# author-hidden-name/GAN-segmentation

Measured on AMD Instinct MI355X. Metric: synthetic (image,mask) pairs/sec, FFHQ-1024 StyleGAN+decoder, higher is better.
Workload: dtype f32; 1 GPU; stylegan-ffhq 1024^2 synthesis + 2-class decoder, batch=8 per GPU, fp32 (BASELINE.json configs[1]); synthetic weights/latents/noise; (img u8, mask u8) resident on rank 0; global_batch=8, parallelism=dp1, gather=none, backend=none, graph=eager (GSA_GRAPH=0)

## Files before the change

### gan-segmentation_amd/csrc/gsa_dev.h

```cpp
#pragma once
#include "gsa_kernels.h"

#ifndef GSA_NO_XCD_REMAP
#define GSA_NO_XCD_REMAP 0
#endif

namespace gsa {

#ifdef GSA_STAMP
#define GSA_DBG_HOOKS 1
#endif
#ifdef GSA_STAMP
#define STAMP(i) do { __builtin_amdgcn_sched_barrier(0); asm volatile("s_memtime %0\n\ts_waitcnt lgkmcnt(0)" : "=s"(stamp_t[i]) :: "memory"); __builtin_amdgcn_sched_barrier(0); } while (0)
#define STAMP_DECL unsigned long long stamp_t[8] = {0, 0, 0, 0, 0, 0, 0, 0}
#define STAMP_FLUSH(nph) do { if (p.stamps && (threadIdx.x & 63) == 0) { for (int i_ = 0; i_ < (nph); ++i_) atomicAdd(&p.stamps[i_], stamp_t[i_ + 1] - stamp_t[i_]); atomicAdd(&p.stamps[15], 1ull); } } while (0)
#define TICK(var) do { __builtin_amdgcn_sched_barrier(0); asm volatile("s_memtime %0\n\ts_waitcnt lgkmcnt(0)" : "=s"(var) :: "memory"); __builtin_amdgcn_sched_barrier(0); } while (0)
#define TSUM(acc, a, b) acc += (b) - (a)
#define TFLUSH(idx, acc) do { if (p.stamps && (threadIdx.x & 63) == 0) atomicAdd(&p.stamps[idx], acc); } while (0)
#else
#define TICK(var) do {} while (0)
#define TSUM(acc, a, b) do {} while (0)
#define TFLUSH(idx, acc) do {} while (0)
#define STAMP(i) do {} while (0)
#define STAMP_DECL do {} while (0)
// ... 99 lines not shown
__device__ __forceinline__ void loads_landed(f32x4 (&r)[2][2]) { asm("" : GSA_LANDED_2(r[0]), GSA_LANDED_2(r[1])); }
__device__ __forceinline__ void loads_landed(f32x4 (&r)[2], f32x4& pin) { asm("" : GSA_LANDED_2(r), "+v"(pin)); }
__device__ __forceinline__ void loads_landed(f32x4 (&r)[3], f32x4& pin) { asm("" : GSA_LANDED_3(r), "+v"(pin)); }
__device__ __forceinline__ void loads_landed(f32x4 (&r)[6], f32x4& pin) { asm("" : GSA_LANDED_6(r), "+v"(pin)); }
__device__ __forceinline__ void loads_landed(f32x4 (&r)[1][2], f32x4& pin) { asm("" : GSA_LANDED_2(r[0]), "+v"(pin)); }
__device__ __forceinline__ void loads_landed(f32x4 (&r)[2][2], f32x4& pin) { asm("" : GSA_LANDED_2(r[0]), GSA_LANDED_2(r[1]), "+v"(pin)); }
__device__ __forceinline__ void vmem_drained(f32x4& pin) {
    asm volatile("" : "+v"(pin));
    __builtin_amdgcn_s_waitcnt(0x0F70);
}
#undef GSA_LANDED_6
#undef GSA_LANDED_3
#undef GSA_LANDED_2
#undef GSA_LANDED_1

__device__ __forceinline__ f32x2 pk_mul2(f32x2 a, f32x2 b) { f32x2 r; asm("v_pk_mul_f32 %0, %1, %2" : "=v"(r) : "v"(a), "v"(b)); return r; }
__device__ __forceinline__ f32x2 pk_mul2_lo(f32x2 a, f32x2 b) { f32x2 r; asm("v_pk_mul_f32 %0, %1, %2 op_sel_hi:[1,0]" : "=v"(r) : "v"(a), "v"(b)); return r; }
__device__ __forceinline__ f32x2 pk_mul2_hi(f32x2 a, f32x2 b) { f32x2 r; asm("v_pk_mul_f32 %0, %1, %2 op_sel:[0,1]" : "=v"(r) : "v"(a), "v"(b)); return r; }
__device__ __forceinline__ f32x4 fma4(const f32x4& a, const f32x4& m, const f32x4& b) {
    const f32x2 lo = fma2v(a.xy, m.xy, b.xy), hi = fma2v(a.zw, m.zw, b.zw);
    return f32x4{lo.x, lo.y, hi.x, hi.y};
}
__device__ __forceinline__ f32x4 lrelu4(const f32x4& v, f32x2 k02) {
    const f32x2 lo = pk_mul2(v.xy, k02), hi = pk_mul2(v.zw, k02);
    return f32x4{max1(v.x, lo.x), max1(v.y, lo.y), max1(v.z, hi.x), max1(v.w, hi.y)};
}

typedef unsigned u32x2 __attribute__((ext_vector_type(2)));

__device__ __forceinline__ float bf16_lo(unsigned u) { return __uint_as_float(u << 16); }
// ... 31 lines not shown
```

### gan-segmentation_amd/csrc/gsa_sub_lean.hip

```cpp
#include "gsa_kernels.h"
#include "gsa_dev.h"

#include <cstdio>
#include <cstdlib>
#include <type_traits>

namespace gsa {
namespace lean {

constexpr int SLW = 10, SRS = SLW * 16 + 4;
constexpr int SIMG = 10 * SRS;
constexpr int SSEG = 16 * 256;
constexpr int STS = 256;

struct STile { int n, y0, x0; };

__device__ __forceinline__ void settle8(f32x4& a, f32x4& b, f32x4& c, f32x4& d, f32x4& e, f32x4& f, f32x4& g, f32x4& h) {
    asm("s_nop 1" : "+v"(a), "+v"(b), "+v"(c), "+v"(d), "+v"(e), "+v"(f), "+v"(g), "+v"(h));
}
__device__ __forceinline__ void settle5(f32x4& a, f32x4& b, f32x4& c, f32x4& d, f32x4& e) { asm("s_nop 1" : "+v"(a), "+v"(b), "+v"(c), "+v"(d), "+v"(e)); }
__device__ __forceinline__ void mfma_settle9(f32x4 (&a)[9]) {
    asm("s_nop 7\n\ts_nop 3" : "+v"(a[0]), "+v"(a[1]), "+v"(a[2]), "+v"(a[3]), "+v"(a[4]), "+v"(a[5]), "+v"(a[6]), "+v"(a[7]), "+v"(a[8]));
}

// ... 80 lines not shown
            const bool aff = AFF && cb < nblk0;
            if (aff) {
                const float* tab = sC + (t.n & 1) * (nblk0 * 32) + cb * 32 + part * 4;
                kA = *reinterpret_cast<const f32x4*>(tab);
                kB = *reinterpret_cast<const f32x4*>(tab + 16);
            }
#pragma unroll
            for (int k = 0; k < 2; ++k) {
                f32x4 v = aff ? fma4(ra[kb][k], kA, kB) : ra[kb][k];
                if (e && ((eflags >> (4 * k)) & (unsigned)e)) v = z;
                if (k == 0 || l_off[1] >= 0) *reinterpret_cast<f32x4*>(img + l_off[k]) = v;
            }
        }
    };

    auto dma_block = [&](int cbk, int slot) {
#pragma unroll
        for (int j = 0; j < 2 * NT; ++j) {
            const int pc = wave8 + 8 * j, q = pc >> 4, r = pc & 15;
            __builtin_amdgcn_global_load_lds((const __attribute__((address_space(1))) void*)(p.wpk + ((size_t)(g * NT + q) * nblk + cbk) * SSEG + r * 256 + lane * 4),
                                             (__attribute__((address_space(3))) void*)(sW + (slot * NT + q) * SSEG + r * 256), 16, 0, 0);
        }
        if (SC && wave8 < NT)
            __builtin_amdgcn_global_load_lds((const __attribute__((address_space(1))) void*)(p.wsc + ((size_t)(g * NT + wave8) * nblk + cbk) * STS + lane * 4),
                                             (__attribute__((address_space(3))) void*)(sS + (slot * NT + wave8) * STS), 16, 0, 0);
    };
    if (WST) {
        dma_block(0, 0);
    } else {
        for (int i = threadIdx.x; i < nblk * NT * (SSEG / 4); i += 512) {
            const int cbk = i / (NT * (SSEG / 4)), r = i % (NT * (SSEG / 4)), q = r / (SSEG / 4), o = r % (SSEG / 4);
            reinterpret_cast<f32x4*>(sW)[i] = reinterpret_cast<const f32x4*>(p.wpk + ((size_t)(g * NT + q) * nblk + cbk) * SSEG)[o];
        }
        if (SC)
            for (int i = threadIdx.x; i < nblk * NT * (STS / 4); i += 512) {
                const int cbk = i / (NT * (STS / 4)), r = i % (NT * (STS / 4)), q = r / (STS / 4), o = r % (STS / 4);
                reinterpret_cast<f32x4*>(sS)[i] = reinterpret_cast<const f32x4*>(p.wsc + ((size_t)(g * NT + q) * nblk + cbk) * STS)[o];
            }
    }
// ... 85 lines not shown
#pragma unroll
                for (int b = 0; b < 2; ++b) {
                    f32x4 v = y[a][b];
                    if (EPI == EPI_DEC) v = lrelu4(fma4(v, e2[nt], e3[nt]), k02);
                    *reinterpret_cast<f32x4*>(ob + ((long)(2 * a) * W + 2 * b) * COUT * 4 + nt * 64 + lane_out) = v;
                }
            if constexpr (SC) {
                char* sb = reinterpret_cast<char*>(p.out_sc) +
                           (((long)(t.n * Hs + (t.y0 >> 1) + (wave >> 1) * 4) * Ws + (t.x0 >> 1) + (wave & 1) * 4) * COUT + g * 16 * NT + nt * 16) * 4;
                f32x4 sv[1] = {accs[nt]};
                asm("s_nop 7\n\ts_nop 3" : "+v"(sv[0]));
                *reinterpret_cast<f32x4*>(sb + lane_sc) = add4(sv[0], scb[nt]);
            }
        }
    };

    STile tc, tr;
    {
        const int w0 = min(w_begin, p.total_tiles - 1);
        const int tx = w0 % p.tiles_x, r = w0 / p.tiles_x;
        tc.x0 = tx * 16; tc.y0 = (r % p.tiles_y) * 16; tc.n = r / p.tiles_y;
    }
    int ec = edge_code(tc), er, cic = 0, cir = 0, n_tab = tc.n;
    auto next_item = [&](STile& t, int& e, int& ci) {
        if (++ci == nitem) { ci = 0; advance(t); e = edge_code(t); }
    };
    if (AFF) fill_coefficients(tc.n);
    if (total_items > 0) load_item(tc, ec, 0);
    if (WST) asm volatile("s_waitcnt vmcnt(0)" ::: "memory");
    if (CNT && t8 < 8) sCnt[t8] = t8 < 4 ? 1u : 0u;
// ... 98 lines not shown
    const int nblk0 = q.C0 / 16, nblk = (q.C0 + q.C1) / 16, wblk = wst ? 2 : nblk;
    return sizeof(float) * ((size_t)wblk * nt * SSEG + (sc ? (size_t)wblk * nt * STS : 0) + 2 * (cnt ? 3 : 2) * kb * SIMG +
                            (aff ? (cnt ? 8 : 2) * 2 * nblk0 * 32 : 0)) + (cnt ? 64 : 0);
}

bool sub_counters(const ConvParams& q, int nt, bool sc, int kb, bool wst) {
#if GSA_EXPERIMENTS
    static const bool cnt_on = env_int("GSA_SUB_CNT", 0) != 0;
    return cnt_on && !wst && sub_lds(q, nt, sc, q.aff0 != nullptr, kb, false, true) <= 160 * 1024;
#else
    (void)q; (void)nt; (void)sc; (void)kb; (void)wst;
    return false;
#endif
}

template <int NT, int EPI, bool SC, bool AFF, int KB, bool WST, bool CNT = false>
hipError_t launch_k(const ConvParams& q, dim3 grid, hipStream_t s) {
    const size_t lds = sub_lds(q, NT, SC, AFF, KB, WST, CNT);
    if (lds > 160 * 1024) return hipErrorInvalidValue;
    return launch<subpixel_lean<NT, EPI, SC, AFF, KB, WST, CNT>>(q.device, grid, dim3(512), lds, s, q);
}

template <int NT, int EPI, bool SC, bool AFF>
hipError_t launch_shape(const ConvParams& q, int kb, bool wst, dim3 grid, hipStream_t s) {
    if (wst) return launch_k<NT, EPI, SC, AFF, 1, true>(q, grid, s);
#if GSA_EXPERIMENTS
    if (sub_counters(q, NT, SC, kb, false))
        return kb == 2 ? launch_k<NT, EPI, SC, AFF, 2, false, true>(q, grid, s) : launch_k<NT, EPI, SC, AFF, 1, false, true>(q, grid, s);
#endif
    return kb == 2 ? launch_k<NT, EPI, SC, AFF, 2, false>(q, grid, s) : launch_k<NT, EPI, SC, AFF, 1, false>(q, grid, s);
}

}

// ... 3 lines not shown
    if (p.aff0 != nullptr && p.C1 != 0) return false;
    return lean::sub_lds(p, nt, sc, p.aff0 != nullptr, kb, wst, false) <= 160 * 1024;
}

hipError_t launch_subpixel_lean(const ConvParams& q, int nt, int epi, bool sc, int kb, bool wst, dim3 grid, hipStream_t s) {
    using namespace lean;
    const bool aff = q.aff0 != nullptr;
#define GSA_SL(NT, EPI, SC) \
    if (nt == NT && epi == EPI && sc == SC) return aff ? launch_shape<NT, EPI, SC, true>(q, kb, wst, grid, s) : launch_shape<NT, EPI, SC, false>(q, kb, wst, grid, s);
    GSA_SL(1, EPI_RAW, false) GSA_SL(2, EPI_RAW, false) GSA_SL(1, EPI_DEC, false) GSA_SL(2, EPI_DEC, false) GSA_SL(1, EPI_DEC, true) GSA_SL(2, EPI_DEC, true)
#undef GSA_SL
    return hipErrorInvalidValue;
}

}
```

### gan-segmentation_amd/csrc/gsa_wino_lean.hip

```cpp
#include "gsa_kernels.h"
#include "gsa_dev.h"

#include <cstdio>
#include <cstdlib>
#include <type_traits>

namespace gsa {
namespace lean {

constexpr int LH = 18, LW = 18, RS = LW * 16 + 4;
constexpr int IMG = LH * RS;
constexpr int SEG = 16 * 256;
constexpr int NPIX = LH * LW;

struct Tile { int n, y0, x0; };

template <int EPI, bool AFF, bool RES, int NB, int GW, bool DB = true, int PF = 1, bool RGB = false>
__global__ __launch_bounds__(256 * GW, GW == 1 ? (DB ? 2 : 3) : 1) void conv3x3_wino_lean(ConvParams p) {
    static_assert(!RGB || (NB == 1 && GW == 1 && DB && AFF && EPI == EPI_DEC), "fused toRGB: the 16 -> 16 decoder kernel with an AdaIN source");
    static_assert(DB || (NB == 1 && GW == 1), "single-buffered form: one block, one group");
    static_assert(PF == 1 || (PF == 2 && DB), "two prefetch sets: the double-buffered form");
    constexpr int NTHR = 256 * GW, CIN = 16 * NB, COUT = 16 * GW;
    constexpr int NCH = (NPIX * 4 + NTHR - 1) / NTHR;
    constexpr bool kLastPartial = (NPIX * 4) % NTHR != 0;
// ... 404 lines not shown
    antiphase_start(p.group_minor, sC);
#endif

    unsigned s_off[NCH], eflags = 0;
    int l_off[NCH];
#pragma unroll
    for (int k = 0; k < NCH; ++k) {
        const int pix = (tid + NTHR * k) >> 2;
        const bool real = pix < NPIX;
        const int ly = real ? pix / LW : 1, lx = real ? pix % LW : 1;
        s_off[k] = (unsigned)(((ly * W + lx) * CIN + part * 4) * 4);
        l_off[k] = real ? ly * RS + lx * 16 + part * 4 : -1;
        eflags |= (unsigned)((ly == 0 ? 1 : 0) | (ly == LH - 1 ? 2 : 0) | (lx == 0 ? 4 : 0) | (lx == LW - 1 ? 8 : 0)) << (4 * k);
    }
    const unsigned safe_off = (unsigned)((((W + 1) * CIN) + part * 4) * 4);
    auto edge_code = [&](const Tile& t) { return (t.y0 == 0 ? 1 : 0) | (t.y0 + 16 == H ? 2 : 0) | (t.x0 == 0 ? 4 : 0) | (t.x0 + 16 == W ? 8 : 0); };
    auto advance = [&](Tile& t) { t.x0 += 16; if (t.x0 == W) { t.x0 = 0; t.y0 += 16; if (t.y0 == H) { t.y0 = 0; t.n += 1; } } };

    f32x4 ra[NCH];
    int dbg_items = 0; (void)dbg_items;
    const float* const wgrp = p.wpk + (size_t)g * NT * nblk * SEG + lane * 4;
    auto dma_weights = [&](int cb, int buf) {
#ifdef GSA_DBG_HOOKS
        if (p.dbg & 16) cb = 0;
        if ((p.dbg & 1024) && dbg_items > 2) return;
#endif
#pragma unroll
        for (int ct = 0; ct < NT; ++ct) {
            const float* wb = wgrp + ((size_t)ct * nblk + cb) * SEG;
#pragma unroll
            for (int j = 0; j < 4; ++j) {
                const int piece = wave + 4 * j;
                __builtin_amdgcn_global_load_lds((const __attribute__((address_space(1))) void*)(wb + piece * 256),
                                                 (__attribute__((address_space(3))) void*)(sB + (PAIR ? buf * 2 + quad : buf * NT + ct) * SEG + piece * 256), 16, 0, 0);
            }
        }
    };
    auto load_item = [&](const Tile& t, int e, int cb) {
        const char* hb = reinterpret_cast<const char*>(p.src0) + ((((long)(t.n * H + t.y0) * W + t.x0) - (W + 1)) * CIN + cb * 16) * 4;
#ifdef GSA_DBG_HOOKS
        if (p.dbg & 32) hb = reinterpret_cast<const char*>(p.src0) + ((long)(W + 1) * CIN) * 4;
        if ((p.dbg & 512) && dbg_items > 2) return;
#endif
        if (e) {
#pragma unroll
            for (int k = 0; k < NCH; ++k) {
                const unsigned bad = (eflags >> (4 * k)) & (unsigned)e;
                const unsigned off = s_off[k] + (bad ? safe_off - s_off[k] : 0u);
                ra[k] = *reinterpret_cast<const f32x4*>(hb + off);
            }
        } else {
#pragma unroll
            for (int k = 0; k < NCH; ++k) ra[k] = *reinterpret_cast<const f32x4*>(hb + s_off[k]);
        }
    };
    int n_coef = -1;
    auto coefficients = [&](int n) {
        __syncthreads();
        for (int e = tid; e < CIN; e += NTHR) {
            const f32x4 a = *reinterpret_cast<const f32x4*>(p.aff0 + (size_t)n * CIN + e);
            sC[(e >> 4) * 32 + (e & 15)] = a[1];
            sC[(e >> 4) * 32 + 16 + (e & 15)] = a[2];
        }
        __syncthreads();
    };
    auto write_item = [&](const Tile& t, int e, int cb, int buf) {
        float* img = sA + buf * IMG;
        if (AFF && t.n != n_coef) { coefficients(t.n); n_coef = t.n; }
#ifdef GSA_DBG_HOOKS
        if (++dbg_items > 2 && (p.dbg & 128)) return;
#endif
        f32x4 kA = {0.f, 0.f, 0.f, 0.f}, kB = kA;
        if (AFF) {
            kA = *reinterpret_cast<const f32x4*>(sC + cb * 32 + part * 4);
            kB = *reinterpret_cast<const f32x4*>(sC + cb * 32 + 16 + part * 4);
        }
        const f32x4 z = {0.f, 0.f, 0.f, 0.f};
        if (e) {
#pragma unroll
            for (int k = 0; k < NCH; ++k) {
                const f32x4 v = AFF ? fma4(ra[k], kA, kB) : ra[k];
                const bool bad = ((eflags >> (4 * k)) & (unsigned)e) != 0;
                if (k < NCH - 1 || l_off[NCH - 1] >= 0) *reinterpret_cast<f32x4*>(img + l_off[k]) = bad ? z : v;
            }
        } else {
#pragma unroll
            for (int k = 0; k < NCH; ++k)
                if (k < NCH - 1 || l_off[NCH - 1] >= 0) *reinterpret_cast<f32x4*>(img + l_off[k]) = AFF ? fma4(ra[k], kA, kB) : ra[k];
        }
    };

    const int wty = ((i16 >> 3) & 1) * 2 + ((i16 >> 1) & 1), wtx = ((i16 >> 2) & 1) * 2 + (i16 & 1);
    const int qy = wave >> 1, qx = wave & 1;
    const int pbase = (qy * 8 + 2 * wty) * RS + (qx * 8 + 2 * wtx) * 16 + kq * 4;
    const int bbase = (kq * 16 + i16) * 4;
    const int co4 = g * NT * 16 + kq * 4;
    const unsigned out_off = (unsigned)((((qy * 8 + 2 * wty) * W + qx * 8 + 2 * wtx) * COUT + co4) * 4);
    if (tid < 16 * NP) {
        float* e = sE + (tid >> 4) * 64 + (tid & 15);
        const int co = (int)blockIdx.y * NP * 16 + tid;
        e[0] = EPI == EPI_SYNTH ? p.nscale[co] : 0.f;
        e[16] = EPI == EPI_SYNTH ? p.nbias[co] : 0.f;
        e[32] = EPI == EPI_DEC ? p.bn_s[co] : 0.f;
        e[48] = EPI == EPI_DEC ? p.bn_beta[co] : 0.f;
    }
    const unsigned nz_off = (unsigned)((((qy * 8 + 2 * wty) * W + qx * 8 + 2 * wtx)) * 4);
    f32x2 nz[2] = {{0.f, 0.f}, {0.f, 0.f}};
    const int s2 = stat_s2(H * W);
    const bool odd = (lane & 1) != 0;
    unsigned long long dI1[NT][4], dI2[NT][4];
#pragma unroll
    for (int ct = 0; ct < NT; ++ct)
#pragma unroll
        for (int c = 0; c < 4; ++c) dI1[ct][c] = dI2[ct][c] = 0ull;
    auto flush_stats = [&](int n) {
#pragma unroll
        for (int ct = 0; ct < NT; ++ct)
#pragma unroll
            for (int c = 0; c < 4; ++c) {
                unsigned long long I1 = dI1[ct][c], I2 = dI2[ct][c];
#pragma unroll
                for (int m = 1; m < 16; m <<= 1) { I1 += shfl_xor_u64(I1, m); I2 += shfl_xor_u64(I2, m); }
                if (i16 == 0) {
                    StatPart* a = p.partials + ((size_t)n * p.prow + (blockIdx.x & (kDirectRows - 1))) * COUT + co4 + ct * 16 + c;
                    atomicAdd(&a->s1, I1);
                    atomicAdd(&a->s2, I2);
                }
                dI1[ct][c] = dI2[ct][c] = 0ull;
            }
    };
    const f32x2 k02 = {0.2f, 0.2f};
    auto epilogue_loads = [&](const Tile& t) {
        if (EPI == EPI_SYNTH) {
            const char* nb = reinterpret_cast<const char*>(p.noise) + ((long)(t.n * H + t.y0) * W + t.x0) * 4;
            nz[0] = *reinterpret_cast<const f32x2*>(nb + nz_off);
            nz[1] = *reinterpret_cast<const f32x2*>(nb + (long)W * 4 + nz_off);
        }
    };

    f32x4 accs[NT][16];
    auto multiply = [&](auto first_tag, int buf, auto&& vm0, auto&& vm1) {
        constexpr bool FIRST = decltype(first_tag)::value;
#ifdef GSA_DBG_HOOKS
        if ((p.dbg & 256) && dbg_items > 2) {
            if (FIRST) for (int ct = 0; ct < NT; ++ct) for (int f = 0; f < 16; ++f) accs[ct][f] = f32x4{0.f, 0.f, 0.f, 0.f};
            return;
        }
#endif
        const float* a_img = sA + buf * IMG + pbase;
        const float* b_img = PAIR ? sB + (buf * 2 + quad) * SEG + bbase : sB + buf * NT * SEG + bbase;
        f32x4 V[16];
#pragma unroll
        for (int c = 0; c < 4; ++c) {
            const f32x4 d0 = *reinterpret_cast<const f32x4*>(a_img + 0 * RS + c * 16);
            const f32x4 d1 = *reinterpret_cast<const f32x4*>(a_img + 1 * RS + c * 16);
            const f32x4 d2 = *reinterpret_cast<const f32x4*>(a_img + 2 * RS + c * 16);
            const f32x4 d3 = *reinterpret_cast<const f32x4*>(a_img + 3 * RS + c * 16);
            V[0 * 4 + c] = sub4(d0, d2);
            V[1 * 4 + c] = add4(d1, d2);
            V[2 * 4 + c] = sub4(d2, d1);
            V[3 * 4 + c] = sub4(d1, d3);
        }
#pragma unroll
        for (int i = 0; i < 4; ++i) {
            const f32x4 t0 = V[i * 4 + 0], t1 = V[i * 4 + 1], t2 = V[i * 4 + 2], t3 = V[i * 4 + 3];
// ... 41 lines not shown
            for (int ct = 0; ct < NT; ++ct)
#pragma unroll
                for (int j = 0; j < 4; ++j) u[ct][j] = *reinterpret_cast<const f32x4*>(b_img + ct * SEG + (fb * 4 + j) * 256);
#pragma unroll
            for (int cg = 0; cg < 4; ++cg)
#pragma unroll
                for (int j = 0; j < 4; ++j)
#pragma unroll
                    for (int ct = 0; ct < NT; ++ct) {
                        const int f = fb * 4 + j;
                        accs[ct][f] = __builtin_amdgcn_mfma_f32_16x16x4f32(u[ct][j][cg], V[f][cg], FIRST && cg == 0 ? f32x4{0.f, 0.f, 0.f, 0.f} : accs[ct][f], 0, 0, 0);
                    }
        }
        __builtin_amdgcn_s_setprio(0);
    };
    auto epilogue_ct = [&](const Tile& t, auto ct_tag) {
        constexpr int ct = decltype(ct_tag)::value;
        f32x4 (&acc)[16] = accs[ct];
        mfma_settle(acc);
        f32x4 s0[4], s1[4];
#pragma unroll
        for (int j = 0; j < 4; ++j) {
            s0[j] = add4(add4(acc[j], acc[4 + j]), acc[8 + j]);
            s1[j] = sub4(sub4(acc[4 + j], acc[8 + j]), acc[12 + j]);
        }
        f32x4 y[2][2];
        y[0][0] = add4(add4(s0[0], s0[1]), s0[2]); y[0][1] = sub4(sub4(s0[1], s0[2]), s0[3]);
        y[1][0] = add4(add4(s1[0], s1[1]), s1[2]); y[1][1] = sub4(sub4(s1[1], s1[2]), s1[3]);
        char* ob = reinterpret_cast<char*>(p.out) + (((long)(t.n * H + t.y0) * W + t.x0) * COUT + ct * 16) * 4;
        const float* sEc = sE + (PAIR ? quad : ct) * 64 + kq * 4;
        const f32x4 e0 = *reinterpret_cast<const f32x4*>(sEc), e1 = *reinterpret_cast<const f32x4*>(sEc + 16);
        const f32x4 e2 = *reinterpret_cast<const f32x4*>(sEc + 32), e3 = *reinterpret_cast<const f32x4*>(sEc + 48);
#pragma unroll
        for (int i = 0; i < 2; ++i)
#pragma unroll
            for (int j = 0; j < 2; ++j) {
                f32x4 v = y[i][j];
                if (EPI == EPI_DEC) v = lrelu4(fma4(v, e2, e3), k02);
                if (EPI == EPI_SYNTH) {
                    const f32x2 tlo = j == 0 ? pk_mul2_lo(e0.xy, nz[i]) : pk_mul2_hi(e0.xy, nz[i]);
                    const f32x2 thi = j == 0 ? pk_mul2_lo(e0.zw, nz[i]) : pk_mul2_hi(e0.zw, nz[i]);
                    v = lrelu4(add4(add4(v, f32x4{tlo.x, tlo.y, thi.x, thi.y}), e1), k02);
                    y[i][j] = v;
                }
#ifdef GSA_DBG_HOOKS
                if (!(p.dbg & 64))
#endif
                *reinterpret_cast<f32x4*>(ob + ((long)i * W + j) * COUT * 4 + out_off) = v;
            }
        if (EPI == EPI_SYNTH) {
            f32x4 ps[2], pq[2];
#pragma unroll
            for (int i = 0; i < 2; ++i) {
                ps[i] = add4(y[i][0], y[i][1]);
                const f32x2 a0 = pk_mul2(y[i][0].xy, y[i][0].xy), a1 = pk_mul2(y[i][0].zw, y[i][0].zw);
                const f32x2 b0 = pk_mul2(y[i][1].xy, y[i][1].xy), b1 = pk_mul2(y[i][1].zw, y[i][1].zw);
                pq[i] = add4(f32x4{a0.x, a0.y, a1.x, a1.y}, f32x4{b0.x, b0.y, b1.x, b1.y});
            }
#pragma unroll
            for (int c = 0; c < 4; ++c) {
                const float keep_s = odd ? ps[1][c] : ps[0][c], send_s = odd ? ps[0][c] : ps[1][c];
                const float keep_q = odd ? pq[1][c] : pq[0][c], send_q = odd ? pq[0][c] : pq[1][c];
                dI1[ct][c] += to_fixed(keep_s + dpp_quad<0xB1>(send_s), kStatScale1);
                dI2[ct][c] += to_fixed_sq(keep_q + dpp_quad<0xB1>(send_q), s2);
            }
        }
    };
    auto epilogue = [&](const Tile& t) {
        epilogue_ct(t, std::integral_constant<int, 0>{});
        if constexpr (NT == 2) epilogue_ct(t, std::integral_constant<int, 1>{});
    };

    Tile tc, tr;
    {
        const int tx = w_begin % p.tiles_x, r = w_begin / p.tiles_x;
        tc.x0 = tx * 16; tc.y0 = (r % p.tiles_y) * 16; tc.n = r / p.tiles_y;
    }
    int ec = edge_code(tc), er, cbc = 0, cbr = 0;
    auto next_item = [&](Tile& t, int& e, int& cb) {
        if (++cb == nblk) { cb = 0; advance(t); e = edge_code(t); }
    };
    dma_weights(0, 0);
    load_item(tc, ec, 0);
    write_item(tc, ec, 0, 0);
    tr = tc; er = ec;
    if (items > 1) {
        next_item(tr, er, cbr);
        load_item(tr, er, cbr);
    }
    __builtin_amdgcn_s_waitcnt(0x0F70);
    __syncthreads();
    unsigned long long k0 = 0, k1 = 0, k2 = 0, k3 = 0, k4 = 0, k5 = 0, sw = 0, sl = 0, sm = 0, se = 0, sb = 0;
    (void)k0; (void)k1; (void)k2; (void)k3; (void)k4; (void)k5; (void)sw; (void)sl; (void)sm; (void)se; (void)sb;
    for (int it = 0; it < items; ++it) {
        const bool has_next = it + 1 < items;
        TICK(k0);
        if (has_next) {
            if (!IL) dma_weights(cbr, (it + 1) & 1);
            write_item(tr, er, cbr, (it + 1) & 1);
        }
        TICK(k1);
        if (cbc == nblk - 1) epilogue_loads(tc);
        Tile t2 = tr; int e2c = er, cb2 = cbr;
        if (it + 2 < items) { next_item(t2, e2c, cb2); if (!IL) load_item(t2, e2c, cb2); }
        TICK(k2);
        auto vm0 = [&]() { if (IL == 1 && has_next) dma_weights(cbr, (it + 1) & 1); };
        auto vm1 = [&]() { if (IL == 1 && it + 2 < items) load_item(t2, e2c, cb2); };
        if (cbc == 0) multiply(std::true_type{}, it & 1, vm0, vm1);
        else multiply(std::false_type{}, it & 1, vm0, vm1);
        vmem_drained(accs[NT - 1][15]);
        TICK(k3);
        if (cbc == nblk - 1) {
            epilogue(tc);
            if (EPI == EPI_SYNTH && (!has_next || tr.n != tc.n)) flush_stats(tc.n);
        }
        TICK(k4);
        __syncthreads();
        TICK(k5);
        TSUM(sw, k0, k1); TSUM(sl, k1, k2); TSUM(sm, k2, k3); TSUM(se, k3, k4); TSUM(sb, k4, k5);
        tc = tr; ec = er; cbc = cbr; tr = t2; er = e2c; cbr = cb2;
    }
    TFLUSH(6, sw); TFLUSH(7, sl); TFLUSH(8, sm); TFLUSH(9, se); TFLUSH(10, sb);
    TFLUSH(12, (unsigned long long)items); TFLUSH(15, 1ull);
}

template <int EPI, bool AFF, int NT = 1, int IL = 0>
__global__ __launch_bounds__(256, NT == 1 ? 2 : 1) void conv3x3_wino_stream(ConvParams p) {
    wino_stream_body<EPI, AFF, NT, IL, false>(p);
}

template <int EPI, bool AFF>
__global__ __launch_bounds__(512, 1) void conv3x3_wino_stream_pair(ConvParams p) {
    wino_stream_body<EPI, AFF, 1, 0, true>(p);
}

template <int EPI, bool AFF, bool RES, int NB, int GW, bool DB = true, int PF = 1, bool RGB = false>
// ... 42 lines not shown
            if (epi == EPI_DEC) {
                if (p.resid) return p.aff0 ? launch_t<EPI_DEC, true, true, 1, 1, true, 2>(p, n, s) : launch_t<EPI_DEC, false, true, 1, 1, true, 2>(p, n, s);
                return p.aff0 ? launch_t<EPI_DEC, true, false, 1, 1, true, 2>(p, n, s) : launch_t<EPI_DEC, false, false, 1, 1, true, 2>(p, n, s);
            }
            if (epi == EPI_SYNTH) return p.aff0 ? launch_t<EPI_SYNTH, true, false, 1, 1, true, 2>(p, n, s) : launch_t<EPI_SYNTH, false, false, 1, 1, true, 2>(p, n, s);
        }
    }
    if (epi == EPI_DEC) {
        if (p.resid) return p.aff0 ? launch_t<EPI_DEC, true, true, NB, GW>(p, n, s) : launch_t<EPI_DEC, false, true, NB, GW>(p, n, s);
        return p.aff0 ? launch_t<EPI_DEC, true, false, NB, GW>(p, n, s) : launch_t<EPI_DEC, false, false, NB, GW>(p, n, s);
    }
    if (epi == EPI_SYNTH) return p.aff0 ? launch_t<EPI_SYNTH, true, false, NB, GW>(p, n, s) : launch_t<EPI_SYNTH, false, false, NB, GW>(p, n, s);
    return hipErrorInvalidValue;
}

template <int EPI, bool AFF, int NT = 1, int IL = 0, bool PAIR = false>
hipError_t launch_stream_t(const ConvParams& p, int n, hipStream_t s) {
    constexpr int NP = PAIR ? 2 : NT;
    const int nblk = p.C0 / 16;
    const size_t lds = sizeof(float) * (2 * IMG + 2 * NP * SEG + 64 * NP + nblk * 32);
    const int cus = device_cus(p.device);
    ConvParams q = p;
    q.wpk = p.wino;
    q.tiles_x = p.W / 16;
    q.tiles_y = p.H / 16;
    q.groups = p.Cout / (16 * NP);
#if GSA_EXPERIMENTS
    static const int stagger = env_int("GSA_STAGGER", 0);
    q.group_minor = PAIR ? 0 : stagger;
#else
    q.group_minor = 0;
#endif
    q.total_tiles = q.tiles_x * q.tiles_y * n;
    if (EPI == EPI_SYNTH) {
// ... 76 lines not shown
        if (wino_stream_paired(p, n)) {
            if (epi == EPI_SYNTH) return p.aff0 ? launch_stream_t<EPI_SYNTH, true, 1, 0, true>(p, n, s) : launch_stream_t<EPI_SYNTH, false, 1, 0, true>(p, n, s);
            if (epi == EPI_DEC) return p.aff0 ? launch_stream_t<EPI_DEC, true, 1, 0, true>(p, n, s) : launch_stream_t<EPI_DEC, false, 1, 0, true>(p, n, s);
            return hipErrorInvalidValue;
        }
        if (epi == EPI_SYNTH) return p.aff0 ? launch_stream_t<EPI_SYNTH, true>(p, n, s) : launch_stream_t<EPI_SYNTH, false>(p, n, s);
        if (epi == EPI_DEC) return p.aff0 ? launch_stream_t<EPI_DEC, true>(p, n, s) : launch_stream_t<EPI_DEC, false>(p, n, s);
        return hipErrorInvalidValue;
    }
    if (p.C0 == 16 && p.Cout == 16) return launch_shape<1, 1>(p, epi, n, s);
    if (p.C0 == 32 && p.Cout == 32) return launch_shape<2, 2>(p, epi, n, s);
    return hipErrorInvalidValue;
}

}
```

Measured before the change: 1427 pairs/s.

## Use incremental 32-bit byte offsets in streaming conv tile walkers

Replaces per-item 64-bit tile address recomputation in the Winograd stream and subpixel weight-stationary kernels with an incremental walker. The walker keeps 32-bit byte offsets, per-sample base pointers and edge/sample flag bits. Weight DMA sources are precomputed per wave, with the block index folded in as a shifted offset. The goal is fewer scalar and vector integer instructions and fewer 64-bit multiplies in the per-block loop. In exchange there is a host-side guard that rejects shapes whose planes exceed the 32-bit offset range, plus more complex state that could mis-address on edge cases.

```diff
diff --git a/gan-segmentation_amd/csrc/gsa_dev.h b/gan-segmentation_amd/csrc/gsa_dev.h
--- a/gan-segmentation_amd/csrc/gsa_dev.h
+++ b/gan-segmentation_amd/csrc/gsa_dev.h
@@ -137,6 +137,15 @@
 #undef GSA_LANDED_2
 #undef GSA_LANDED_1
 
+__device__ __forceinline__ unsigned lane_offset(unsigned off) {
+    asm volatile("" : "+v"(off));
+    return off;
+}
+
+inline bool plane_fits_u32(long rows, long cols, long channels) {
+    return rows > 0 && cols > 0 && channels > 0 && (unsigned long long)(rows + 2) * (unsigned long long)cols * (unsigned long long)channels * 4ull < (1ull << 32);
+}
+
 __device__ __forceinline__ f32x2 pk_mul2(f32x2 a, f32x2 b) { f32x2 r; asm("v_pk_mul_f32 %0, %1, %2" : "=v"(r) : "v"(a), "v"(b)); return r; }
 __device__ __forceinline__ f32x2 pk_mul2_lo(f32x2 a, f32x2 b) { f32x2 r; asm("v_pk_mul_f32 %0, %1, %2 op_sel_hi:[1,0]" : "=v"(r) : "v"(a), "v"(b)); return r; }
 __device__ __forceinline__ f32x2 pk_mul2_hi(f32x2 a, f32x2 b) { f32x2 r; asm("v_pk_mul_f32 %0, %1, %2 op_sel:[0,1]" : "=v"(r) : "v"(a), "v"(b)); return r; }
diff --git a/gan-segmentation_amd/csrc/gsa_sub_lean.hip b/gan-segmentation_amd/csrc/gsa_sub_lean.hip
--- a/gan-segmentation_amd/csrc/gsa_sub_lean.hip
+++ b/gan-segmentation_amd/csrc/gsa_sub_lean.hip
@@ -118,15 +118,21 @@
         }
     };
 
+    const char* wsrc[NT];
+#pragma unroll
+    for (int q = 0; q < NT; ++q) wsrc[q] = reinterpret_cast<const char*>(p.wpk + ((size_t)(g * NT + q) * nblk) * SSEG + wave8 * 256);
+    const char* const wscb = reinterpret_cast<const char*>(p.wsc) + (SC && wave8 < NT ? ((size_t)(g * NT + wave8) * nblk) * STS * sizeof(float) : 0);
+    const unsigned lane16 = (unsigned)lane * 16u;
     auto dma_block = [&](int cbk, int slot) {
+        const unsigned voff = lane16 + ((unsigned)cbk << 14), voff8 = voff + 8192u;
 #pragma unroll
         for (int j = 0; j < 2 * NT; ++j) {
             const int pc = wave8 + 8 * j, q = pc >> 4, r = pc & 15;
-            __builtin_amdgcn_global_load_lds((const __attribute__((address_space(1))) void*)(p.wpk + ((size_t)(g * NT + q) * nblk + cbk) * SSEG + r * 256 + lane * 4),
+            __builtin_amdgcn_global_load_lds((const __attribute__((address_space(1))) void*)(wsrc[j >> 1] + ((j & 1) ? voff8 : voff)),
                                              (__attribute__((address_space(3))) void*)(sW + (slot * NT + q) * SSEG + r * 256), 16, 0, 0);
         }
         if (SC && wave8 < NT)
-            __builtin_amdgcn_global_load_lds((const __attribute__((address_space(1))) void*)(p.wsc + ((size_t)(g * NT + wave8) * nblk + cbk) * STS + lane * 4),
+            __builtin_amdgcn_global_load_lds((const __attribute__((address_space(1))) void*)(wscb + (lane16 + ((unsigned)cbk << 10))),
                                              (__attribute__((address_space(3))) void*)(sS + (slot * NT + wave8) * STS), 16, 0, 0);
     };
     if (WST) {
@@ -242,6 +248,190 @@
             }
         }
     };
+
+    if constexpr (WST) {
+        constexpr unsigned kSample = 16u, kSlot = 32u;
+        struct Walk { int tx, ty, cb; unsigned s0, s1, m; };
+        const int tx_last = p.tiles_x - 1, ty_last = p.tiles_y - 1;
+        const unsigned px0 = (unsigned)p.C0 * 4u, px1 = (unsigned)p.C1 * 4u, px_out = (unsigned)COUT * 4u;
+        const unsigned wrap0 = 7u * (unsigned)Ws * px0, wrap1 = 7u * (unsigned)Ws * px1;
+        const unsigned plane0 = (unsigned)(Hs * Ws) * px0, plane1 = (unsigned)(Hs * Ws) * px1;
+        auto edge_of = [&](const Walk& w) { return (w.ty == 0 ? 1u : 0u) | (w.ty == ty_last ? 2u : 0u) | (w.tx == 0 ? 4u : 0u) | (w.tx == tx_last ? 8u : 0u); };
+        Walk wl;
+        int n_cur;
+        {
+            const int w0 = min(w_begin, p.total_tiles - 1);
+            const int tx = w0 % p.tiles_x, r = w0 / p.tiles_x;
+            wl.tx = tx; wl.ty = r % p.tiles_y; wl.cb = 0; n_cur = r / p.tiles_y;
+            const unsigned tpix = (unsigned)(wl.ty * 8 * Ws + tx * 8);
+            wl.s0 = tpix * px0; wl.s1 = tpix * px1;
+            wl.m = edge_of(wl) | ((n_cur & 1) ? kSlot : 0u);
+        }
+        const char* b0 = reinterpret_cast<const char*>(p.src0) + (size_t)n_cur * (size_t)plane0 - (size_t)(Ws + 1) * px0;
+        const char* b1 = reinterpret_cast<const char*>(p.src1) + (size_t)n_cur * (size_t)plane1 - (size_t)(Ws + 1) * px1;
+        const char* affb = reinterpret_cast<const char*>(p.aff0) + (AFF ? (size_t)n_cur * p.C0 * sizeof(Aff) : 0);
+        char* outb;
+        char* scout;
+        auto sample_bases = [&](int n) {
+            outb = reinterpret_cast<char*>(p.out) + ((size_t)n * H * W + py * W + px) * px_out + g * 16 * NT * 4;
+            scout = reinterpret_cast<char*>(p.out_sc) + (SC ? ((size_t)n * Hs * Ws + (wave >> 1) * 4 * Ws + (wave & 1) * 4) * px_out + g * 16 * NT * 4 : 0);
+        };
+        sample_bases(n_cur);
+        auto next_item_w = [&](Walk& w) {
+            ++w.cb;
+            w.m &= ~kSample;
+            if (w.cb == nblk) {
+                unsigned m = w.m & kSlot;
+                w.cb = 0;
+                w.s0 += 8u * px0; w.s1 += 8u * px1;
+                if (w.tx == tx_last) {
+                    w.tx = 0;
+                    w.s0 += wrap0; w.s1 += wrap1;
+                    if (w.ty == ty_last) { w.ty = 0; w.s0 = w.s1 = 0u; b0 += (size_t)plane0; b1 += (size_t)plane1; m = (m ^ kSlot) | kSample; }
+                    else ++w.ty;
+                } else ++w.tx;
+                w.m = m | edge_of(w);
+            }
+        };
+        unsigned pixo[2];
+#pragma unroll
+        for (int k = 0; k < 2; ++k) {
+            const int pix = (t8 + 256 * k) >> 2;
+            const bool real = pix < 100;
+            pixo[k] = (unsigned)((real ? pix / SLW : 1) * Ws + (real ? pix % SLW : 1));
+        }
+        const unsigned part16 = (unsigned)part * 16u, safe_px = lane_offset((unsigned)(Ws + 1));
+        auto load_item_w = [&](const Walk& w) {
+            const unsigned e = w.m & 15u;
+            const bool first = w.cb < nblk0;
+            const char* hb = first ? b0 + (w.s0 + ((unsigned)w.cb << 6)) : b1 + (w.s1 + ((unsigned)(w.cb - nblk0) << 6));
+            const unsigned cpx = first ? px0 : px1;
+#pragma unroll
+            for (int k = 0; k < 2; ++k) {
+                const unsigned real_off = __umul24(pixo[k], cpx) + part16, safe = __umul24(safe_px, cpx) + part16;
+                const unsigned bad = (eflags >> (4 * k)) & e;
+                ra[0][k] = *reinterpret_cast<const f32x4*>(hb + (real_off + (bad ? safe - real_off : 0u)));
+            }
+        };
+        auto fill_coefficients_w = [&](unsigned m) {
+            float* tab = sC + ((m & kSlot) ? nblk0 * 32 : 0);
+            for (unsigned eo = (unsigned)t8 * 16u; eo < (unsigned)p.C0 * 16u; eo += 4096u) {
+                const f32x4 a = *reinterpret_cast<const f32x4*>(affb + lane_offset(eo));
+                const unsigned e = eo >> 4;
+                tab[(e >> 4) * 32 + (e & 15)] = a[1];
+                tab[(e >> 4) * 32 + 16 + (e & 15)] = a[2];
+            }
+            affb += (size_t)p.C0 * sizeof(Aff);
+        };
+        auto write_item_w = [&](unsigned m, int cb, int a_off) {
+            const f32x4 z = {0.f, 0.f, 0.f, 0.f};
+            const unsigned e = m & 15u;
+            float* img = sA + a_off;
+            f32x4 kA = z, kB = z;
+            const bool aff = AFF && cb < nblk0;
+            if (aff) {
+                const float* tab = sC + ((m & kSlot) ? nblk0 * 32 : 0) + cb * 32 + part * 4;
+                kA = *reinterpret_cast<const f32x4*>(tab);
+                kB = *reinterpret_cast<const f32x4*>(tab + 16);
+            }
+#pragma unroll
+            for (int k = 0; k < 2; ++k) {
+                f32x4 v = aff ? fma4(ra[0][k], kA, kB) : ra[0][k];
+                if (e && ((eflags >> (4 * k)) & e)) v = z;
+                if (k == 0 || l_off[1] >= 0) *reinterpret_cast<f32x4*>(img + l_off[k]) = v;
+            }
+        };
+        auto epilogue_w = [&](unsigned txy) {
+            const unsigned ty = txy >> 16, tx = txy & 0xffffu;
+            char* ob = outb + (ty * 16u * (unsigned)W + tx * 16u) * px_out;
+            const unsigned lo = lane_offset(lane_out);
+#pragma unroll
+            for (int nt = 0; nt < NT; ++nt) {
+                f32x4 m[9];
+#pragma unroll
+                for (int f = 0; f < 9; ++f) m[f] = acc[f][nt];
+                mfma_settle9(m);
+                f32x4 s0[3], s1[3], y[2][2];
+#pragma unroll
+                for (int j = 0; j < 3; ++j) { s0[j] = add4(m[j], m[3 + j]); s1[j] = add4(m[3 + j], m[6 + j]); }
+                y[0][0] = add4(s0[0], s0[1]); y[0][1] = add4(s0[1], s0[2]);
+                y[1][0] = add4(s1[0], s1[1]); y[1][1] = add4(s1[1], s1[2]);
+#pragma unroll
+                for (int a = 0; a < 2; ++a)
+#pragma unroll
+                    for (int b = 0; b < 2; ++b) {
+                        f32x4 v = y[a][b];
+                        if (EPI == EPI_DEC) v = lrelu4(fma4(v, e2[nt], e3[nt]), k02);
+                        *reinterpret_cast<f32x4*>(ob + (unsigned)(2 * a * W + 2 * b) * px_out + nt * 64 + lo) = v;
+                    }
+                if constexpr (SC) {
+                    char* sb = scout + (ty * 8u * (unsigned)Ws + tx * 8u) * px_out + nt * 64;
+                    f32x4 sv[1] = {accs[nt]};
+                    asm("s_nop 7\n\ts_nop 3" : "+v"(sv[0]));
+                    *reinterpret_cast<f32x4*>(sb + lane_offset(lane_sc)) = add4(sv[0], scb[nt]);
+                }
+            }
+        };
+
+        unsigned m_r = 0u, txy_c = (unsigned)wl.ty << 16 | (unsigned)wl.tx, txy_r = 0u;
+        int cb_c = 0, cbn = 0, a_cur = 0, slot = 0;
+        if (AFF) fill_coefficients_w(wl.m);
+        if (total_items > 0) load_item_w(wl);
+        asm volatile("s_waitcnt vmcnt(0)" ::: "memory");
+        __syncthreads();
+        if (total_items > 0) write_item_w(wl.m, 0, 0);
+        if (total_items > 1) {
+            next_item_w(wl);
+            if (AFF && (wl.m & kSample)) fill_coefficients_w(wl.m);
+            load_item_w(wl);
+            m_r = wl.m; txy_r = (unsigned)wl.ty << 16 | (unsigned)wl.tx;
+        }
+        loads_landed(ra);
+        __syncthreads();
+        unsigned long long k0 = 0, k1 = 0, k2 = 0, k3 = 0, k4 = 0, k5 = 0, sw = 0, sl = 0, sm = 0, se = 0, sb = 0;
+        (void)k0; (void)k1; (void)k2; (void)k3; (void)k4; (void)k5; (void)sw; (void)sl; (void)sm; (void)se; (void)sb;
+        auto trip = [&](auto steady_tag, int it) {
+            constexpr bool STEADY = decltype(steady_tag)::value;
+            const bool ring = STEADY || it + 1 < iters, active = STEADY || it < total_items;
+            const bool has_next = STEADY || it + 1 < total_items, has_load = STEADY || it + 2 < total_items;
+            TICK(k0);
+            cbn = cbn + 1 == nblk ? 0 : cbn + 1;
+            if (ring) dma_block(cbn, slot ^ 1);
+            if (active) {
+                if (has_next) write_item_w(m_r, cbn, a_cur ^ SIMG);
+                TICK(k1);
+                if (has_load) {
+                    next_item_w(wl);
+                    if (AFF && (wl.m & kSample)) fill_coefficients_w(wl.m);
+                    load_item_w(wl);
+                }
+                TICK(k2);
+                if (cb_c == 0) mfma_block(std::true_type{}, sA + a_cur, slot);
+                else mfma_block(std::false_type{}, sA + a_cur, slot);
+                vmem_drained(acc[8][NT - 1]);
+                TICK(k3);
+                if (cb_c == nblk - 1) {
+                    epilogue_w(txy_c);
+                    if (!has_next || (m_r & kSample)) sample_bases(++n_cur);
+                }
+                TICK(k4);
+                cb_c = cbn; txy_c = txy_r;
+                if (has_load) { m_r = wl.m; txy_r = (unsigned)wl.ty << 16 | (unsigned)wl.tx; }
+            } else {
+                __builtin_amdgcn_s_waitcnt(0x0F70);
+            }
+            __syncthreads();
+            TICK(k5);
+            if (active) { TSUM(sw, k0, k1); TSUM(sl, k1, k2); TSUM(sm, k2, k3); TSUM(se, k3, k4); TSUM(sb, k4, k5); }
+            a_cur ^= SIMG; slot ^= 1;
+        };
+        int it = 0;
+        for (; it + 2 < total_items; ++it) trip(std::true_type{}, it);
+        for (; it < iters; ++it) trip(std::false_type{}, it);
+        TFLUSH(6, sw); TFLUSH(7, sl); TFLUSH(8, sm); TFLUSH(9, se); TFLUSH(10, sb);
+        TFLUSH(12, (unsigned long long)total_items); TFLUSH(15, 1ull);
+        return;
+    }
 
     STile tc, tr;
     {
@@ -370,10 +560,15 @@
 #endif
 }
 
+bool sub_offsets_fit(int Hs, int Ws, int C0, int C1, int Cout) {
+    return plane_fits_u32(Hs, Ws, C0) && (C1 == 0 || plane_fits_u32(Hs, Ws, C1)) && plane_fits_u32(2L * Hs, 2L * Ws, Cout);
+}
+
 template <int NT, int EPI, bool SC, bool AFF, int KB, bool WST, bool CNT = false>
 hipError_t launch_k(const ConvParams& q, dim3 grid, hipStream_t s) {
     const size_t lds = sub_lds(q, NT, SC, AFF, KB, WST, CNT);
     if (lds > 160 * 1024) return hipErrorInvalidValue;
+    if (WST && !sub_offsets_fit(q.Hs, q.Ws, q.C0, q.C1, q.Cout)) return hipErrorInvalidValue;
     return launch<subpixel_lean<NT, EPI, SC, AFF, KB, WST, CNT>>(q.device, grid, dim3(512), lds, s, q);
 }
 
@@ -407,3 +602,5 @@
 }
 
 }
+
+extern "C" int gsa_subpixel_stream_offsets_fit(int Hs, int Ws, int C0, int C1, int Cout) { return gsa::lean::sub_offsets_fit(Hs, Ws, C0, C1, Cout) ? 1 : 0; }
diff --git a/gan-segmentation_amd/csrc/gsa_wino_lean.hip b/gan-segmentation_amd/csrc/gsa_wino_lean.hip
--- a/gan-segmentation_amd/csrc/gsa_wino_lean.hip
+++ b/gan-segmentation_amd/csrc/gsa_wino_lean.hip
@@ -442,30 +442,77 @@
         eflags |= (unsigned)((ly == 0 ? 1 : 0) | (ly == LH - 1 ? 2 : 0) | (lx == 0 ? 4 : 0) | (lx == LW - 1 ? 8 : 0)) << (4 * k);
     }
     const unsigned safe_off = (unsigned)((((W + 1) * CIN) + part * 4) * 4);
-    auto edge_code = [&](const Tile& t) { return (t.y0 == 0 ? 1 : 0) | (t.y0 + 16 == H ? 2 : 0) | (t.x0 == 0 ? 4 : 0) | (t.x0 + 16 == W ? 8 : 0); };
-    auto advance = [&](Tile& t) { t.x0 += 16; if (t.x0 == W) { t.x0 = 0; t.y0 += 16; if (t.y0 == H) { t.y0 = 0; t.n += 1; } } };
+
+    constexpr unsigned kSample = 16u;
+    struct Walk { int tx, ty, cb; unsigned src, pix, m; };
+    const int tx_last = p.tiles_x - 1, ty_last = p.tiles_y - 1;
+    const unsigned px_src = (unsigned)CIN * 4u, px_out = (unsigned)COUT * 4u;
+    const unsigned tile_src = 15u * px_src;
+    const unsigned wrap_pix = 15u * (unsigned)W, wrap_src = wrap_pix * px_src;
+    const size_t plane_src = (size_t)H * W * px_src;
+    Walk wl;
+    int n_cur;
+    {
+        const int tx = w_begin % p.tiles_x, r = w_begin / p.tiles_x;
+        wl.tx = tx; wl.ty = r % p.tiles_y; wl.cb = 0; n_cur = r / p.tiles_y;
+        wl.pix = (unsigned)(wl.ty * 16 * W + tx * 16);
+        wl.src = wl.pix * px_src;
+        wl.m = (wl.ty == 0 ? 1u : 0u) | (wl.ty == ty_last ? 2u : 0u) | (tx == 0 ? 4u : 0u) | (tx == tx_last ? 8u : 0u);
+    }
+    const char* srcb = reinterpret_cast<const char*>(p.src0) + (size_t)n_cur * plane_src - (size_t)(W + 1) * px_src;
+    char* outb;
+    const char* nzb;
+    auto sample_bases = [&](int n) {
+        outb = reinterpret_cast<char*>(p.out) + (size_t)n * H * W * px_out;
+        nzb = reinterpret_cast<const char*>(p.noise) + (EPI == EPI_SYNTH ? (size_t)n * H * W * 4 : 0);
+    };
+    sample_bases(n_cur);
+    const char* affb = reinterpret_cast<const char*>(p.aff0) + (AFF ? (size_t)n_cur * CIN * sizeof(Aff) : 0);
+    auto next_item = [&](Walk& w) {
+        ++w.cb; w.src += 64u;
+        w.m &= 15u;
+        if (w.cb == nblk) {
+            unsigned m = 0u;
+            w.cb = 0;
+            w.src += tile_src; w.pix += 16u;
+            if (w.tx == tx_last) {
+                w.tx = 0;
+                w.src += wrap_src; w.pix += wrap_pix;
+                if (w.ty == ty_last) { w.ty = 0; w.src = w.pix = 0u; srcb += plane_src; m |= kSample; }
+                else ++w.ty;
+            } else ++w.tx;
+            w.m = m | (w.ty == 0 ? 1u : 0u) | (w.ty == ty_last ? 2u : 0u) | (w.tx == 0 ? 4u : 0u) | (w.tx == tx_last ? 8u : 0u);
+        }
+    };
 
     f32x4 ra[NCH];
     int dbg_items = 0; (void)dbg_items;
-    const float* const wgrp = p.wpk + (size_t)g * NT * nblk * SEG + lane * 4;
-    auto dma_weights = [&](int cb, int buf) {
+    const char* wsrc[NT][4];
+#pragma unroll
+    for (int ct = 0; ct < NT; ++ct)
+#pragma unroll
+        for (int j = 0; j < 4; ++j) wsrc[ct][j] = reinterpret_cast<const char*>(p.wpk + ((size_t)(g * NT + ct) * nblk) * SEG + (wave + 4 * j) * 256);
+    const unsigned lane16 = (unsigned)lane * 16u;
+    int a_cur = 0, b_cur = 0;
+    auto dma_weights = [&](int cb, int b_off) {
 #ifdef GSA_DBG_HOOKS
         if (p.dbg & 16) cb = 0;
         if ((p.dbg & 1024) && dbg_items > 2) return;
 #endif
+        const unsigned voff = lane16 + ((unsigned)cb << 14);
 #pragma unroll
         for (int ct = 0; ct < NT; ++ct) {
-            const float* wb = wgrp + ((size_t)ct * nblk + cb) * SEG;
 #pragma unroll
             for (int j = 0; j < 4; ++j) {
                 const int piece = wave + 4 * j;
-                __builtin_amdgcn_global_load_lds((const __attribute__((address_space(1))) void*)(wb + piece * 256),
-                                                 (__attribute__((address_space(3))) void*)(sB + (PAIR ? buf * 2 + quad : buf * NT + ct) * SEG + piece * 256), 16, 0, 0);
-            }
-        }
-    };
-    auto load_item = [&](const Tile& t, int e, int cb) {
-        const char* hb = reinterpret_cast<const char*>(p.src0) + ((((long)(t.n * H + t.y0) * W + t.x0) - (W + 1)) * CIN + cb * 16) * 4;
+                __builtin_amdgcn_global_load_lds((const __attribute__((address_space(1))) void*)(wsrc[ct][j] + voff),
+                                                 (__attribute__((address_space(3))) void*)(sB + b_off + (PAIR ? quad : ct) * SEG + piece * 256), 16, 0, 0);
+            }
+        }
+    };
+    auto load_item = [&](const Walk& w) {
+        const unsigned e = w.m & 15u;
+        const char* hb = srcb + w.src;
 #ifdef GSA_DBG_HOOKS
         if (p.dbg & 32) hb = reinterpret_cast<const char*>(p.src0) + ((long)(W + 1) * CIN) * 4;
         if ((p.dbg & 512) && dbg_items > 2) return;
@@ -482,19 +529,21 @@
             for (int k = 0; k < NCH; ++k) ra[k] = *reinterpret_cast<const f32x4*>(hb + s_off[k]);
         }
     };
-    int n_coef = -1;
-    auto coefficients = [&](int n) {
+    auto coefficients = [&]() {
         __syncthreads();
-        for (int e = tid; e < CIN; e += NTHR) {
-            const f32x4 a = *reinterpret_cast<const f32x4*>(p.aff0 + (size_t)n * CIN + e);
+        for (unsigned eo = (unsigned)tid * 16u; eo < (unsigned)CIN * 16u; eo += NTHR * 16u) {
+            const f32x4 a = *reinterpret_cast<const f32x4*>(affb + lane_offset(eo));
+            const unsigned e = eo >> 4;
             sC[(e >> 4) * 32 + (e & 15)] = a[1];
             sC[(e >> 4) * 32 + 16 + (e & 15)] = a[2];
         }
         __syncthreads();
-    };
-    auto write_item = [&](const Tile& t, int e, int cb, int buf) {
-        float* img = sA + buf * IMG;
-        if (AFF && t.n != n_coef) { coefficients(t.n); n_coef = t.n; }
+        affb += (size_t)CIN * sizeof(Aff);
+    };
+    auto write_item = [&](unsigned m, int cb, int a_off) {
+        float* img = sA + a_off;
+        const unsigned e = m & 15u;
+        if (AFF && (m & kSample)) coefficients();
 #ifdef GSA_DBG_HOOKS
         if (++dbg_items > 2 && (p.dbg & 128)) return;
 #endif
@@ -524,6 +573,9 @@
     const int bbase = (kq * 16 + i16) * 4;
     const int co4 = g * NT * 16 + kq * 4;
     const unsigned out_off = (unsigned)((((qy * 8 + 2 * wty) * W + qx * 8 + 2 * wtx) * COUT + co4) * 4);
+    unsigned nz_off[2];
+#pragma unroll
+    for (int i = 0; i < 2; ++i) nz_off[i] = (unsigned)((((qy * 8 + 2 * wty + i) * W + qx * 8 + 2 * wtx)) * 4);
     if (tid < 16 * NP) {
         float* e = sE + (tid >> 4) * 64 + (tid & 15);
         const int co = (int)blockIdx.y * NP * 16 + tid;
@@ -532,7 +584,6 @@
         e[32] = EPI == EPI_DEC ? p.bn_s[co] : 0.f;
         e[48] = EPI == EPI_DEC ? p.bn_beta[co] : 0.f;
     }
-    const unsigned nz_off = (unsigned)((((qy * 8 + 2 * wty) * W + qx * 8 + 2 * wtx)) * 4);
     f32x2 nz[2] = {{0.f, 0.f}, {0.f, 0.f}};
     const int s2 = stat_s2(H * W);
     const bool odd = (lane & 1) != 0;
@@ -558,16 +609,16 @@
             }
     };
     const f32x2 k02 = {0.2f, 0.2f};
-    auto epilogue_loads = [&](const Tile& t) {
+    auto epilogue_loads = [&](unsigned pix) {
         if (EPI == EPI_SYNTH) {
-            const char* nb = reinterpret_cast<const char*>(p.noise) + ((long)(t.n * H + t.y0) * W + t.x0) * 4;
-            nz[0] = *reinterpret_cast<const f32x2*>(nb + nz_off);
-            nz[1] = *reinterpret_cast<const f32x2*>(nb + (long)W * 4 + nz_off);
+            const char* nb = nzb + (pix << 2);
+            nz[0] = *reinterpret_cast<const f32x2*>(nb + lane_offset(nz_off[0]));
+            nz[1] = *reinterpret_cast<const f32x2*>(nb + lane_offset(nz_off[1]));
         }
     };
 
     f32x4 accs[NT][16];
-    auto multiply = [&](auto first_tag, int buf, auto&& vm0, auto&& vm1) {
+    auto multiply = [&](auto first_tag, int a_off, int b_off, auto&& vm0, auto&& vm1) {
         constexpr bool FIRST = decltype(first_tag)::value;
 #ifdef GSA_DBG_HOOKS
         if ((p.dbg & 256) && dbg_items > 2) {
@@ -575,8 +626,8 @@
             return;
         }
 #endif
-        const float* a_img = sA + buf * IMG + pbase;
-        const float* b_img = PAIR ? sB + (buf * 2 + quad) * SEG + bbase : sB + buf * NT * SEG + bbase;
+        const float* a_img = sA + a_off + pbase;
+        const float* b_img = sB + b_off + (PAIR ? quad * SEG : 0) + bbase;
         f32x4 V[16];
 #pragma unroll
         for (int c = 0; c < 4; ++c) {
@@ -648,7 +699,7 @@
         }
         __builtin_amdgcn_s_setprio(0);
     };
-    auto epilogue_ct = [&](const Tile& t, auto ct_tag) {
+    auto epilogue_ct = [&](unsigned pix, auto ct_tag) {
         constexpr int ct = decltype(ct_tag)::value;
         f32x4 (&acc)[16] = accs[ct];
         mfma_settle(acc);
@@ -661,7 +712,9 @@
         f32x4 y[2][2];
         y[0][0] = add4(add4(s0[0], s0[1]), s0[2]); y[0][1] = sub4(sub4(s0[1], s0[2]), s0[3]);
         y[1][0] = add4(add4(s1[0], s1[1]), s1[2]); y[1][1] = sub4(sub4(s1[1], s1[2]), s1[3]);
-        char* ob = reinterpret_cast<char*>(p.out) + (((long)(t.n * H + t.y0) * W + t.x0) * COUT + ct * 16) * 4;
+        char* ob = outb + pix * px_out + ct * 64;
+        const unsigned px_row = (unsigned)W * px_out;
+        const unsigned lo = lane_offset(out_off);
         const float* sEc = sE + (PAIR ? quad : ct) * 64 + kq * 4;
         const f32x4 e0 = *reinterpret_cast<const f32x4*>(sEc), e1 = *reinterpret_cast<const f32x4*>(sEc + 16);
         const f32x4 e2 = *reinterpret_cast<const f32x4*>(sEc + 32), e3 = *reinterpret_cast<const f32x4*>(sEc + 48);
@@ -680,7 +733,7 @@
 #ifdef GSA_DBG_HOOKS
                 if (!(p.dbg & 64))
 #endif
-                *reinterpret_cast<f32x4*>(ob + ((long)i * W + j) * COUT * 4 + out_off) = v;
+                *reinterpret_cast<f32x4*>(ob + (i * px_row + j * px_out) + lo) = v;
             }
         if (EPI == EPI_SYNTH) {
             f32x4 ps[2], pq[2];
@@ -700,60 +753,59 @@
             }
         }
     };
-    auto epilogue = [&](const Tile& t) {
-        epilogue_ct(t, std::integral_constant<int, 0>{});
-        if constexpr (NT == 2) epilogue_ct(t, std::integral_constant<int, 1>{});
-    };
-
-    Tile tc, tr;
-    {
-        const int tx = w_begin % p.tiles_x, r = w_begin / p.tiles_x;
-        tc.x0 = tx * 16; tc.y0 = (r % p.tiles_y) * 16; tc.n = r / p.tiles_y;
-    }
-    int ec = edge_code(tc), er, cbc = 0, cbr = 0;
-    auto next_item = [&](Tile& t, int& e, int& cb) {
-        if (++cb == nblk) { cb = 0; advance(t); e = edge_code(t); }
-    };
+    auto epilogue = [&](unsigned pix) {
+        epilogue_ct(pix, std::integral_constant<int, 0>{});
+        if constexpr (NT == 2) epilogue_ct(pix, std::integral_constant<int, 1>{});
+    };
+
+    unsigned pix_c = wl.pix, m_r = 0u, pix_r = 0u;
+    int cb_c = 0, cb_r = 0;
     dma_weights(0, 0);
-    load_item(tc, ec, 0);
-    write_item(tc, ec, 0, 0);
-    tr = tc; er = ec;
+    load_item(wl);
+    write_item(wl.m | kSample, 0, 0);
     if (items > 1) {
-        next_item(tr, er, cbr);
-        load_item(tr, er, cbr);
+        next_item(wl);
+        load_item(wl);
+        m_r = wl.m; cb_r = wl.cb; pix_r = wl.pix;
     }
     __builtin_amdgcn_s_waitcnt(0x0F70);
     __syncthreads();
     unsigned long long k0 = 0, k1 = 0, k2 = 0, k3 = 0, k4 = 0, k5 = 0, sw = 0, sl = 0, sm = 0, se = 0, sb = 0;
     (void)k0; (void)k1; (void)k2; (void)k3; (void)k4; (void)k5; (void)sw; (void)sl; (void)sm; (void)se; (void)sb;
-    for (int it = 0; it < items; ++it) {
-        const bool has_next = it + 1 < items;
+    auto body = [&](auto next_tag, auto load_tag) {
+        const bool HAS_NEXT = next_tag, HAS_LOAD = load_tag;
+        const int a_nxt = a_cur ^ IMG, b_nxt = b_cur ^ (NP * SEG);
         TICK(k0);
-        if (has_next) {
-            if (!IL) dma_weights(cbr, (it + 1) & 1);
-            write_item(tr, er, cbr, (it + 1) & 1);
+        if (HAS_NEXT) {
+            if (!IL) dma_weights(cb_r, b_nxt);
+            write_item(m_r, cb_r, a_nxt);
         }
         TICK(k1);
-        if (cbc == nblk - 1) epilogue_loads(tc);
-        Tile t2 = tr; int e2c = er, cb2 = cbr;
-        if (it + 2 < items) { next_item(t2, e2c, cb2); if (!IL) load_item(t2, e2c, cb2); }
+        if (cb_c == nblk - 1) epilogue_loads(pix_c);
+        if (HAS_LOAD) { next_item(wl); if (!IL) load_item(wl); }
         TICK(k2);
-        auto vm0 = [&]() { if (IL == 1 && has_next) dma_weights(cbr, (it + 1) & 1); };
-        auto vm1 = [&]() { if (IL == 1 && it + 2 < items) load_item(t2, e2c, cb2); };
-        if (cbc == 0) multiply(std::true_type{}, it & 1, vm0, vm1);
-        else multiply(std::false_type{}, it & 1, vm0, vm1);
+        auto vm0 = [&]() { if (IL == 1 && HAS_NEXT) dma_weights(cb_r, b_nxt); };
+        auto vm1 = [&]() { if (IL == 1 && HAS_LOAD) load_item(wl); };
+        if (cb_c == 0) multiply(std::true_type{}, a_cur, b_cur, vm0, vm1);
+        else multiply(std::false_type{}, a_cur, b_cur, vm0, vm1);
         vmem_drained(accs[NT - 1][15]);
         TICK(k3);
-        if (cbc == nblk - 1) {
-            epilogue(tc);
-            if (EPI == EPI_SYNTH && (!has_next || tr.n != tc.n)) flush_stats(tc.n);
+        if (cb_c == nblk - 1) {
+            epilogue(pix_c);
+            if (!HAS_NEXT || (m_r & kSample)) {
+                if (EPI == EPI_SYNTH) flush_stats(n_cur);
+                sample_bases(++n_cur);
+            }
         }
         TICK(k4);
         __syncthreads();
         TICK(k5);
         TSUM(sw, k0, k1); TSUM(sl, k1, k2); TSUM(sm, k2, k3); TSUM(se, k3, k4); TSUM(sb, k4, k5);
-        tc = tr; ec = er; cbc = cbr; tr = t2; er = e2c; cbr = cb2;
-    }
+        cb_c = cb_r; pix_c = pix_r;
+        if (HAS_LOAD) { m_r = wl.m; cb_r = wl.cb; pix_r = wl.pix; }
+        a_cur = a_nxt; b_cur = b_nxt;
+    };
+    for (int it = 0; it < items; ++it) body(it + 1 < items, it + 2 < items);
     TFLUSH(6, sw); TFLUSH(7, sl); TFLUSH(8, sm); TFLUSH(9, se); TFLUSH(10, sb);
     TFLUSH(12, (unsigned long long)items); TFLUSH(15, 1ull);
 }
@@ -826,10 +878,13 @@
     return hipErrorInvalidValue;
 }
 
+bool stream_offsets_fit(int H, int W, int Cin, int Cout) { return plane_fits_u32(H, W, Cin) && plane_fits_u32(H, W, Cout); }
+
 template <int EPI, bool AFF, int NT = 1, int IL = 0, bool PAIR = false>
 hipError_t launch_stream_t(const ConvParams& p, int n, hipStream_t s) {
     constexpr int NP = PAIR ? 2 : NT;
     const int nblk = p.C0 / 16;
+    if (!stream_offsets_fit(p.H, p.W, p.C0, p.Cout)) return hipErrorInvalidValue;
     const size_t lds = sizeof(float) * (2 * IMG + 2 * NP * SEG + 64 * NP + nblk * 32);
     const int cus = device_cus(p.device);
     ConvParams q = p;
@@ -936,3 +991,5 @@
 }
 
 }
+
+extern "C" int gsa_wino_stream_offsets_fit(int H, int W, int Cin, int Cout) { return gsa::lean::stream_offsets_fit(H, W, Cin, Cout) ? 1 : 0; }
```

Result: no change. 1437 pairs/s, median of 6 (+0.8%).
